# dschrempf/mcmc-date

Measured on AMD Instinct MI355X. Metric: MVN log-likelihood evals/sec (= MCMC steps/sec × chains) at N=256 nodes, higher is better.
Workload: dtype f64; 1 GPU; synthetic 256-dimensional MVN (dense random SPD Sigma, seed 256), 512 chains per GPU, kind=logpdf; n=256, chains_per_gpu=512, kernel=logpdf, launch=hipGraph replay, swap_period=0, parallelism=chains sharded x1, no data-path collective, form=sweep

## Files before the change

mcmc-date_amd/csrc/k_logpdf.hip:

```cpp
#include "mvn_device.hpp"
#include "stripe_device.hpp"

namespace mcd {

template <int R, int BT, int CW, int LW, int FS>
__global__ void __launch_bounds__(64 * (CW + LW)) k_logpdf(const double* __restrict__ F, const double* __restrict__ mu,
                                                           const double* __restrict__ invdiag, const double* __restrict__ X, int64_t ldx,
                                                           int64_t batch, int n, int ncols, double* __restrict__ ll, double c, double logdet)
{
    MCD_KERNEL_HEAD_FS(FS)
    MCD_ACC_DECL
    MCD_T(0);
    if (wave >= CW) {
        const int lw = wave - CW;
        fwd_loader_role<R, LW, FS>(F, ring, lw, lane, ncols MCD_ACC_ARGS);
        MCD_T(3);
        MCD_ACC_FLUSH(5);
        return;
    }
    const MvnView M(mu, invdiag, n, c, logdet);
    double d[R][BT];
    load_rawx<R, BT, FS == 2>(d, M, X, ldx, b0, batch, lane);
    MCD_T(1);
    lds_barrier();
// ... 2 lines not shown
    MCD_T(3);
    finish_ll<R, BT>(d, M, b0, batch, ll, lane);
    MCD_T(4);
    MCD_ACC_FLUSH(5);
}

template <int R, int S, bool SH, int SC>
__global__ void __launch_bounds__(64 * S) k_logpdf_stripe(const double* __restrict__ Fw, const double* __restrict__ mu,
                                                          const double* __restrict__ invdiag, const double* __restrict__ X, int64_t ldx,
                                                          int64_t batch, int n, int ncols, double* __restrict__ ll, double c, double logdet)
{
    __shared__ d2 ring[SH ? Stripe<R, S>::D3 : Stripe<R, S>::D2];
    const int lane = threadIdx.x & 63;
    const int wave = __builtin_amdgcn_readfirstlane(threadIdx.x >> 6);
    MCD_T(0);
    const MvnView M(mu, invdiag, n, c, logdet);
    stripe_dispatch<R, S, 0, SH, SC>(wave, Fw, ring, M, X, ldx, (int64_t)blockIdx.x * 2, batch, ncols, ll, lane);
}

template <int R, int S>
__global__ void __launch_bounds__(64 * S) k_logpdf_stripe_fin(const double* __restrict__ Fw, const double* __restrict__ mu,
                                                              const double* __restrict__ invdiag, const double* __restrict__ X, int64_t ldx,
                                                              int64_t batch, int n, int ncols, double* __restrict__ ll, double c, double logdet)
{
    static_assert(kStripeArgC == 8 * 8, "c follows Fw, mu, invdiag, X, ldx, batch, {n, ncols} and ll");
    __shared__ d2 ring[Stripe<R, S>::D3];
    const int lane = threadIdx.x & 63;
    const int wave = __builtin_amdgcn_readfirstlane(threadIdx.x >> 6);
    MCD_T(0);
    const MvnView M(mu, invdiag, n, 0.0, 0.0);
    stripe_dispatch_fin<R, S, 0>(wave, Fw, ring, M, X, ldx, (int64_t)blockIdx.x * 2, batch, ncols, ll, lane);
}

template <int R, bool SH, int SC>
static void launch_stripe_sh(const MvnDev& M, const double* X, int64_t ldx, int64_t batch, double* ll, hipStream_t st)
{
    hipLaunchKernelGGL((k_logpdf_stripe<R, kStripeWaves, SH, SC>), dim3((unsigned)((batch + 1) / 2)), dim3(64 * kStripeWaves), 0, st, M.Fw, M.mu,
                       M.invdiag, X, ldx, batch, M.n, M.ncols, ll, M.c, M.logdet);
}
template <int R>
static void launch_stripe(const MvnDev& M, const double* X, int64_t ldx, int64_t batch, double* ll, hipStream_t st)
{
    const int pro = opt_or(OPT_STRIPE_PROLOGUE, kStripePrologueDefault), sched = opt_or(OPT_STRIPE_SCHED, kStripeSchedDefault);
    const int sc = stripe_schedule(pro, sched, R, M.ncols);
    if (sc < 0) launch_stripe_sh<R, false, 0>(M, X, ldx, batch, ll, st);
    else if (stripe_finish(pro, sched, opt_or(OPT_STRIPE_FINISH, kStripeFinishDefault), R, M.ncols) != 0)
        hipLaunchKernelGGL((k_logpdf_stripe_fin<R, kStripeWaves>), dim3((unsigned)((batch + 1) / 2)), dim3(64 * kStripeWaves), 0, st, M.Fw, M.mu,
                           M.invdiag, X, ldx, batch, M.n, M.ncols, ll, M.c, M.logdet);
    else if (sc == 2) launch_stripe_sh<R, true, 2>(M, X, ldx, batch, ll, st);
    else if (sc == 1) launch_stripe_sh<R, true, 1>(M, X, ldx, batch, ll, st);
    else launch_stripe_sh<R, true, 0>(M, X, ldx, batch, ll, st);
}

template <int R, int BT, int CW, int LW, int FS>
static void launch_fs(const MvnDev& M, const double* X, int64_t ldx, int64_t batch, double* ll, hipStream_t st)
{
    const int64_t per_wg = (int64_t)CW * BT;
    const unsigned grid = (unsigned)((batch + per_wg - 1) / per_wg);
    hipLaunchKernelGGL((k_logpdf<R, BT, CW, LW, FS>), dim3(grid), dim3(64 * (CW + LW)), 0, st, fwd_stream_ptr(M, FS), M.mu, M.invdiag, X, ldx,
                       batch, M.n, M.ncols, ll, M.c, M.logdet);
}

template <int R, int BT, int CW, int LW>
static void launch_geom(const MvnDev& M, const double* X, int64_t ldx, int64_t batch, double* ll, hipStream_t st)
{
    if constexpr (fwd_stream_compact(R)) {
        constexpr bool INV = CW == 2 && BT == 1;
        const int fs = fwd_stream<R>(CW, INV, INV && logpdf_inverse_window(MvnFacts(M), batch));
        if (fs == 1) return launch_fs<R, BT, CW, LW, 1>(M, X, ldx, batch, ll, st);
        if (fs == 2) return launch_fs<R, BT, CW, LW, 2>(M, X, ldx, batch, ll, st);
        if constexpr (INV)
            if (fs == 3) return launch_stripe<R>(M, X, ldx, batch, ll, st);
    }
    launch_fs<R, BT, CW, LW, 0>(M, X, ldx, batch, ll, st);
}

template <int R>
static hipError_t launch_logpdf_R(const MvnDev& M, const double* X, int64_t ldx, int64_t batch, double* ll, hipStream_t st)
{
// ... 40 lines not shown
```

mcmc-date_amd/csrc/mvn_capi.cpp:

```cpp
#include <hip/hip_runtime.h>

#include <cmath>
#include <cstdarg>
#include <cstdio>
#include <cstring>
#include <memory>
#include <mutex>
#include <string>
#include <vector>

#include "../../include/mcmcdate_mvn.h"
#include "fc_layout.hpp"
#include "host_factor.h"
#include "mvn_kernels.h"

namespace {

thread_local std::string g_last_error;

int fail(int code, const char* fmt, ...)
{
    char buf[512];
    va_list ap;
    va_start(ap, fmt);
// ... 207 lines not shown
        mcd::invert_factor(n, h->L, W);
    }
    h->n = n;
    h->R = mcd::padded_blocks(n);
    h->device = device_id;
    if (h->R < 0) return fail(MCD_ERR_UNSUPPORTED, "mcd_mvn_create: unsupported dimension %d", n);
    if (mat_kind == MCD_MAT_SIGMA_INV) {
        h->logdet = logdet_sigma;
    } else {
        double s = 0.0;
        for (int i = 0; i < n; ++i) s += std::log(h->L[(size_t)i * n + i]);
        h->logdet = 2.0 * s;
    }
    std::vector<double> mu_pad, invdiag, Ft, Ut;
    mcd::pack_factors(n, h->R, h->L, mu_pad, mu, invdiag, Ft, Ut);

    HIP_TRY(hipSetDevice(device_id));
    const size_t NP = (size_t)64 * h->R;
    HIP_TRY(hipMalloc((void**)&h->d_mu, NP * sizeof(double)));
    HIP_TRY(hipMalloc((void**)&h->d_invdiag, NP * sizeof(double)));
    HIP_TRY(hipMalloc((void**)&h->d_Ft, NP * NP * sizeof(double)));
    HIP_TRY(hipMalloc((void**)&h->d_Ut, NP * NP * sizeof(double)));
    HIP_TRY(hipMemcpy(h->d_mu, mu_pad.data(), NP * sizeof(double), hipMemcpyHostToDevice));
    HIP_TRY(hipMemcpy(h->d_invdiag, invdiag.data(), NP * sizeof(double), hipMemcpyHostToDevice));
    HIP_TRY(hipMemcpy(h->d_Ft, Ft.data(), NP * NP * sizeof(double), hipMemcpyHostToDevice));
    HIP_TRY(hipMemcpy(h->d_Ut, Ut.data(), NP * NP * sizeof(double), hipMemcpyHostToDevice));
    if (mcd::fwd_stream_compact(h->R)) {
        std::vector<double> Fc;
        mcd::pack_compact_forward(h->R, Ft, Fc);
        HIP_TRY(hipMalloc((void**)&h->d_Fc, Fc.size() * sizeof(double)));
        HIP_TRY(hipMemcpy(h->d_Fc, Fc.data(), Fc.size() * sizeof(double), hipMemcpyHostToDevice));
        std::vector<double> Fw;
        mcd::pack_inverse_forward(n, h->R, W, Fw);
        HIP_TRY(hipMalloc((void**)&h->d_Fw, Fw.size() * sizeof(double)));
        HIP_TRY(hipMemcpy(h->d_Fw, Fw.data(), Fw.size() * sizeof(double), hipMemcpyHostToDevice));
    }

    const int ch = mcd::sweep_chunk_columns(h->R);
    h->dev.n = n;
    h->dev.R = h->R;
    h->dev.ncols = ((n + ch - 1) / ch) * ch;
    h->dev.c = -(0.9189385332046727417803297364056176 * (double)n);
    h->dev.logdet = h->logdet;
    h->dev.mu = h->d_mu;
    h->dev.invdiag = h->d_invdiag;
    h->dev.Ft = h->d_Ft;
    h->dev.Fc = h->d_Fc;
    h->dev.Fw = h->d_Fw;
    h->dev.Ut = h->d_Ut;
    {
        std::vector<double> Wt, Wtb;
        mcd::pack_w_tiles(n, W, Wt, Wtb);
        HIP_TRY(hipMalloc((void**)&h->d_Wt, Wt.size() * sizeof(double)));
        HIP_TRY(hipMemcpy(h->d_Wt, Wt.data(), Wt.size() * sizeof(double), hipMemcpyHostToDevice));
        HIP_TRY(hipMalloc((void**)&h->d_Wtb, Wtb.size() * sizeof(double)));
        HIP_TRY(hipMemcpy(h->d_Wtb, Wtb.data(), Wtb.size() * sizeof(double), hipMemcpyHostToDevice));
        h->dev.Wt = h->d_Wt;
        h->dev.Wtb = h->d_Wtb;
        if (h->R >= 1) {
            std::vector<double> Wc((size_t)n * NP, 0.0);
            for (int j = 0; j < n; ++j)
                for (int i = j; i < n; ++i) Wc[(size_t)j * NP + i] = W[(size_t)i * n + j];
            HIP_TRY(hipMalloc((void**)&h->d_Wc, Wc.size() * sizeof(double)));
            HIP_TRY(hipMemcpy(h->d_Wc, Wc.data(), Wc.size() * sizeof(double), hipMemcpyHostToDevice));
            h->dev.Wc = h->d_Wc;
        }
        HIP_TRY(mcd::prepare_wide());
        HIP_TRY(mcd::prepare_wide_grad());
// ... 307 lines not shown
```

mcmc-date_amd/csrc/options.cpp:

```cpp
#include "options.h"

#include <atomic>
#include <cstdlib>
#include <cstring>

#include "../../include/mcmcdate_mvn.h"

extern "C" int mcd_set_last_error_(int code, const char* msg);

namespace mcd {
namespace {

const char* const kNames[OPT_COUNT] = {
    "MCD_MH_PER_PHASE", "MCD_MH_SEGMENTS", "MCD_MH_INCREMENTAL", "MCD_MH_PRIOR", "MCD_MH_PRIOR_CACHE", "MCD_MH_STEP_WG", "MCD_MH_CHAIN_LW",
    "MCD_MH_INC_SLOTS", "MCD_MH_SPARSE_SLOTS", "MCD_SPLIT", "MCD_SPLIT_G", "MCD_SPLIT_SCATTER", "MCD_SPLIT_NOROT", "MCD_SPLIT_PROBE", "MCD_GEOM",
    "MCD_WIDE_CT", "MCD_SPARSE_QUAD", "MCD_MH_PRIOR_WAVES", "MCD_LOADERS", "MCD_MH_SEG_TAIL", "MCD_MH_AHEAD_FROM", "MCD_MH_PRIOR_DRAWS",
    "MCD_FSTREAM", "MCD_SPARSE_GRAD_CHAINS", "MCD_STRIPE_PROLOGUE", "MCD_STRIPE_SCHED", "MCD_STRIPE_FINISH"};

struct Table {
    std::atomic<int> v[OPT_COUNT];
    Table()
    {
        for (int i = 0; i < OPT_COUNT; ++i) {
            const char* e = std::getenv(kNames[i]);
            v[i].store((e && *e) ? std::atoi(e) : MCD_OPT_UNSET, std::memory_order_relaxed);
        }
    }
};
Table& table()
{
    static Table t;
    return t;
}
const Table& g_seed_at_load = table();

int find(const char* name)
{
    if (!name) return -1;
    for (int i = 0; i < OPT_COUNT; ++i)
        if (std::strcmp(name, kNames[i]) == 0) return i;
    return -1;
}

}

int opt_get(Option o) { return table().v[o].load(std::memory_order_relaxed); }

namespace {
thread_local unsigned long long t_last_lds = 0;
}
// ... 27 lines not shown
```

mcmc-date_amd/csrc/options.h:

```cpp
#pragma once

namespace mcd {

enum Option {
    OPT_MH_PER_PHASE = 0,
    OPT_MH_SEGMENTS,
    OPT_MH_INCREMENTAL,
    OPT_MH_PRIOR,
    OPT_MH_PRIOR_CACHE,
    OPT_MH_STEP_WG,
    OPT_MH_CHAIN_LW,
    OPT_MH_INC_SLOTS,
    OPT_MH_SPARSE_SLOTS,
    OPT_SPLIT,
    OPT_SPLIT_G,
    OPT_SPLIT_SCATTER,
    OPT_SPLIT_NOROT,
    OPT_SPLIT_PROBE,
    OPT_GEOM,
    OPT_WIDE_CT,
    OPT_SPARSE_QUAD,
    OPT_MH_PRIOR_WAVES,
    OPT_LOADERS,
    OPT_MH_SEG_TAIL,
    OPT_MH_AHEAD_FROM,
    OPT_MH_PRIOR_DRAWS,
    OPT_FSTREAM,
    OPT_SPARSE_GRAD_CHAINS,
    OPT_STRIPE_PROLOGUE,
    OPT_STRIPE_SCHED,
    OPT_STRIPE_FINISH,
    OPT_COUNT
};
constexpr int MCD_OPT_UNSET = -2147483647 - 1;

int opt_get(Option o);
void note_dynamic_lds(unsigned long long bytes);
unsigned long long last_dynamic_lds();
inline bool opt_is(Option o, int v) { return opt_get(o) == v; }
inline int opt_or(Option o, int dflt) { const int v = opt_get(o); return v == MCD_OPT_UNSET ? dflt : v; }

}
```

mcmc-date_amd/csrc/stripe_device.hpp:

```cpp
#pragma once
#include "mvn_device.hpp"
#include "stripe_deal.hpp"
#include "stripe_plan.hpp"

namespace mcd {

#ifndef MCD_STRIPE_WAVES
#define MCD_STRIPE_WAVES 4
#endif
constexpr int kStripeWaves = MCD_STRIPE_WAVES;
#ifndef MCD_STRIPE_AHEAD
#define MCD_STRIPE_AHEAD 12
#endif
constexpr int kStripeAhead = MCD_STRIPE_AHEAD;

template <int R, int S>
struct Stripe {
    static_assert((R == 3 || R == 4) && (S == 4 || S == 8), "stripe kernel: R = 3, 4; S = 4, 8");
    static constexpr int D = 128 / S;
    static constexpr int A = kStripeAhead < D ? kStripeAhead : D;
    static_assert(A >= 1, "MCD_STRIPE_AHEAD");
    static constexpr int ZERO = S * D * 64;
    static constexpr int D2 = ZERO + S * 64;
    static constexpr int EXCH = D2;
// ... 544 lines not shown
        }
    }
    MCD_T(1);
}

template <int R, int S, int W, int I, int NO>
__device__ __forceinline__ void stripe_exchange_put(const double (&xr)[NO + 1][2], const double (&m)[NO + 1], const double (&iv)[NO + 1], unsigned ea,
                                                    int n, int64_t b0, int64_t batch, int lane)
{
    if constexpr (I < NO) {
        constexpr int k = W + I * S;
        const int row = 64 * k + lane;
        double rr[2], tt[2];
#pragma unroll
        for (int c = 0; c < 2; ++c) {
            const double xv = (row < n && b0 + c < batch) ? xr[I][c] : m[I];
            rr[c] = xv - m[I];
            tt[c] = rr[c] * iv[I];
        }
        lds_write16<k * 1024>(ea, d2{rr[0], rr[1]});
        lds_write16<(R + k) * 1024>(ea, d2{tt[0], tt[1]});
        stripe_exchange_put<R, S, W, I + 1, NO>(xr, m, iv, ea, n, b0, batch, lane);
    }
}
template <int R, int Q, int K>
__device__ __forceinline__ void stripe_exchange_get(d2 (&e)[R], unsigned ea)
{
    if constexpr (K < R) {
        lds_read16<(Q * R + K) * 1024>(e[K], ea);
        stripe_exchange_get<R, Q, K + 1>(e, ea);
    }
}

template <int R, int S, int W, bool GETR = true, class Burst>
__device__ __forceinline__ void stripe_prologue_shared(unsigned ea, const MvnView& M, const double* __restrict__ X, int64_t ldx, int64_t b0,
                                                       int64_t batch, double (&r)[R][2], double (&a)[R][2], int lane, Burst burst)
{
    using G = Stripe<R, S>;
    constexpr int PRO = stripe_min(G::A, G::T.n[W]);
    constexpr int NO = W < R ? (R - W + S - 1) / S : 0;
    double xr[NO + 1][2], m[NO + 1], iv[NO + 1];
#pragma unroll
    for (int i = 0; i < NO; ++i) {
        const int row = 64 * (W + i * S) + lane;
        asm_load8(m[i], M.mu + row);
        asm_load8(iv[i], M.invdiag + row);
        const int rc = row < M.n ? row : M.n - 1;
#pragma unroll
        for (int c = 0; c < 2; ++c) {
            const int64_t bc = (b0 + c < batch) ? b0 + c : batch - 1;
            asm_load8(xr[i][c], X + bc * ldx + rc);
        }
    }
    burst();
    asm_wait_vmcnt<PRO>();
#pragma unroll
    for (int i = 0; i < NO; ++i) asm volatile("" : "+v"(m[i]), "+v"(iv[i]), "+v"(xr[i][0]), "+v"(xr[i][1]));
    MCD_T(1);
    stripe_exchange_put<R, S, W, 0, NO>(xr, m, iv, ea, M.n, b0, batch, lane);
    lds_barrier();
    d2 e[R], et[R];
    if constexpr (GETR) stripe_exchange_get<R, 0, 0>(e, ea);
    if constexpr (W == 0) stripe_exchange_get<R, 1, 0>(et, ea);
    if constexpr (GETR) lds_landed<R>(e);
    if constexpr (W == 0) lds_landed<R>(et);
#pragma unroll
    for (int k = 0; k < R; ++k)
#pragma unroll
        for (int c = 0; c < 2; ++c) {
            if constexpr (GETR) r[k][c] = c ? e[k].y : e[k].x;
            if constexpr (W == 0) a[k][c] = c ? et[k].y : et[k].x;
            else a[k][c] = 0.0;
// ... 48 lines not shown
            const double* pw = reinterpret_cast<const double*>(ring + w * D * 64);
#pragma unroll
            for (int k = 0; k < R; ++k)
#pragma unroll
                for (int c = 0; c < 2; ++c) a[k][c] = a[k][c] + pw[(k * 2 + c) * 64 + lane];
        }
        finish_ll<R, 2>(a, M, b0, batch, ll, lane);
        MCD_T(4);
    }
}

#ifndef MCD_STRIPE_FINISH_WAVE
#define MCD_STRIPE_FINISH_WAVE 0
#endif
constexpr int kStripeFinishWave = MCD_STRIPE_FINISH_WAVE;
constexpr int kStripeArgC = 0x40;
typedef unsigned stripe_u4 __attribute__((ext_vector_type(4)));
__device__ __forceinline__ void stripe_args_load(stripe_u4& v)
{
#if defined(__HIP_DEVICE_COMPILE__)
    asm volatile("s_load_dwordx4 %0, %1, %2" : "=&s"(v) : "s"(__builtin_amdgcn_kernarg_segment_ptr()), "n"(kStripeArgC) : "memory");
#endif
}
__device__ __forceinline__ void stripe_args_landed(stripe_u4& v)
{
    asm volatile("s_waitcnt lgkmcnt(0)" : "+s"(v)::"memory");
}
template <int OFF>
__device__ __forceinline__ void lds_read8(double& v, unsigned addr)
{
    static_assert(OFF >= 0 && OFF < 65536, "ds offset");
    asm volatile("ds_read_b64 %0, %1 offset:%2" : "=v"(v) : "v"(addr), "n"(OFF) : "memory");
}
template <int R, int S, int W, int C, int I>
__device__ __forceinline__ void stripe_finish_get(double (&p)[S][R], unsigned pa)
{
    if constexpr (I < S * R) {
        constexpr int w = I / R, k = I % R;
        if constexpr (w != W) lds_read8<(k * 2 + C) * 512>(p[w][k], pa + (unsigned)(w * Stripe<R, S>::D * 1024));
        stripe_finish_get<R, S, W, C, I + 1>(p, pa);
    }
}
template <int R, int S, int W, int C>
__device__ __forceinline__ void stripe_finish_chain(const double (&a)[R][2], unsigned pa, stripe_u4& cl, int64_t b0, int64_t batch,
                                                    double* __restrict__ ll, int lane)
{
    double p[S][R];
    stripe_finish_get<R, S, W, C, 0>(p, pa);
    asm volatile("s_waitcnt lgkmcnt(0)" ::: "memory");
#pragma unroll
    for (int w = 0; w < S; ++w)
#pragma unroll
        for (int k = 0; k < R; ++k)
            if (w != W) asm volatile("" : "+v"(p[w][k]));
    MCD_T(7);
    double s = 0.0;
#pragma unroll
    for (int k = 0; k < R; ++k) {
        double z = W == 0 ? a[k][C] : p[0][k];
#pragma unroll
        for (int w = 1; w < S; ++w) z = z + (w == W ? a[k][C] : p[w][k]);
        s = fma(z, z, s);
    }
    const double q = wave_sum(s);
    stripe_args_landed(cl);
    const double c = __hiloint2double((int)cl.y, (int)cl.x), logdet = __hiloint2double((int)cl.w, (int)cl.z);
    if (lane == 0 && b0 + C < batch) ll[b0 + C] = c + (-0.5) * (logdet + q);
}

template <int R, int S, int W>
__device__ __forceinline__ void stripe_wave_fin(const double* __restrict__ Fw, d2* ring, const MvnView& M, const double* __restrict__ X, int64_t ldx,
                                                int64_t b0, int64_t batch, int ncols, double* __restrict__ ll, int lane)
{
    using G = Stripe<R, S>;
    static_assert(kStripeFinishWave >= 0 && kStripeFinishWave + 2 <= S, "MCD_STRIPE_FINISH_WAVE");
    constexpr int D = G::D, NU = G::T.n[W], PRO = stripe_min(G::A, NU);
    constexpr int C = W - kStripeFinishWave;
    constexpr bool FIN = C == 0 || C == 1;
    stripe_u4 cl;
    if constexpr (FIN) stripe_args_load(cl);
    d2* my = ring + W * D * 64;
// ... 15 lines not shown
    for (int k = 0; k < R; ++k)
#pragma unroll
        for (int c = 0; c < 2; ++c)
            if (c != C) part[(k * 2 + c) * 64 + lane] = a[k][c];
    lds_barrier();
    if constexpr (FIN) {
        MCD_T(6);
        stripe_finish_chain<R, S, W, C>(a, lds_addr(ring) + 8u * (unsigned)lane, cl, b0, batch, ll, lane);
        MCD_T(4);
    }
}
template <int R, int S, int W>
__device__ __forceinline__ void stripe_dispatch_fin(int wave, const double* __restrict__ Fw, d2* ring, const MvnView& M, const double* __restrict__ X,
                                                    int64_t ldx, int64_t b0, int64_t batch, int ncols, double* __restrict__ ll, int lane)
{
    if (wave == W) {
        stripe_wave_fin<R, S, W>(Fw, ring, M, X, ldx, b0, batch, ncols, ll, lane);
    } else {
        if constexpr (W + 1 < S) stripe_dispatch_fin<R, S, W + 1>(wave, Fw, ring, M, X, ldx, b0, batch, ncols, ll, lane);
    }
}

template <int R, int S, int W, bool SH, int SC>
__device__ __forceinline__ void stripe_dispatch(int wave, const double* __restrict__ Fw, d2* ring, const MvnView& M, const double* __restrict__ X,
                                                int64_t ldx, int64_t b0, int64_t batch, int ncols, double* __restrict__ ll, int lane)
{
    if (wave == W) {
        stripe_wave<R, S, W, SH, SC>(Fw, ring, M, X, ldx, b0, batch, ncols, ll, lane);
    } else {
        if constexpr (W + 1 < S) stripe_dispatch<R, S, W + 1, SH, SC>(wave, Fw, ring, M, X, ldx, b0, batch, ncols, ll, lane);
    }
}

}
```

mcmc-date_amd/csrc/stripe_plan.hpp:

```cpp
#pragma once

#include "stripe_deal.hpp"

namespace mcd {

constexpr int kStripeRegSlots = 24;
constexpr int kStripeMaxGroups = 32;
constexpr int kStripeBaseSpan = 8192, kStripeBaseBias = 4096;

struct StripePlan {
    int n, lead, pro, D, A;
    int kind[kStripeMaxUnits];
    int slot[kStripeMaxUnits];
    int base[kStripeMaxUnits];
    int imm[kStripeMaxUnits];
    int group[kStripeMaxUnits];
    int ng;
    int gci[kStripeMaxGroups], gdiag[kStripeMaxGroups];
    int gbeg[kStripeMaxGroups], gend[kStripeMaxGroups];
    int gpre[kStripeMaxGroups];
    int gwait[kStripeMaxGroups];
    int gpost[kStripeMaxGroups];
};

// ... 97 lines not shown
        issued = upto;
    };
    issue(p.pro, -1, -1);
    if (p.lead + issued >= 64) return 3;
    for (int g = 0; g < p.ng && !fail; ++g) {
        issue(p.gpre[g], g - 2, g - 1);
        if (issued - landed >= 64) return 3;
        if (issued < p.gend[g] || p.gwait[g] != issued - p.gend[g] || p.gwait[g] > 63) return 2;
        landed = p.gend[g];
        issue(p.gpost[g], g - 1, g);
        if (issued - landed >= 64) return 3;
    }
    if (fail) return fail;
    return issued == p.n ? 0 : 8;
}

constexpr bool stripe_plans_cover(int R, int S, int A)
{
    int seen[256] = {};
    const StripeDeal d = stripe_deal(R, S);
    for (int w = 0; w < S; ++w) {
        const StripePlan p = stripe_plan(R, S, w, A);
        if (stripe_plan_check(p, R, S, w) != 0) return false;
        for (int u = 0; u < p.n; ++u) {
            const int unit = p.kind[u] ? (p.base[u] + p.imm[u]) / 1024 : d.unit[w][u];
            if (unit < 0 || unit >= fc_total_units(R) || seen[unit]++) return false;
        }
    }
    for (int i = 0; i < fc_total_units(R); ++i)
        if (seen[i] != 1) return false;
    return true;
}

}
```

mcmc-date_amd/csrc/sweep_launch.cpp:

```cpp
#include "sweep_groups.hpp"
#include "stripe_deal.hpp"
#include "stripe_plan.hpp"
#include <stdlib.h>
#include <atomic>

namespace mcd {

int sweep_chunk_columns(int R)
{
    return 2 * ((R == 1) ? 32 : (R == 2) ? 16 : (R <= 4) ? 8 : 4);
}

int wide_chain_tiles(int64_t batch)
{
    const int force = opt_or(OPT_WIDE_CT, 0);
    if (force == 1 || force == 2 || force == 4) return force;
    return batch <= 256 * 16 ? 1 : 2;
}

static std::atomic<int> g_form{getenv("MCD_WIDE") ? (atoi(getenv("MCD_WIDE")) ? 2 : 1) : 0};

int set_logpdf_form(int form) { return g_form.exchange(form); }

int effective_form(const MvnDev& M)
// ... 216 lines not shown
    if ((R != 3 && R != 4) || (S != 4 && S != 8) || w < 0 || w >= S) return -1;
    const mcd::StripeDeal d = mcd::stripe_deal(R, S);
    int np = 0;
    auto put = [&](int ci, int p, int pos, int units) {
        if (np < cap) {
            int* q = piece + 5 * np;
            q[0] = ci, q[1] = p, q[2] = d.unit[w][pos], q[3] = units, q[4] = pos;
        }
        ++np;
    };
    for (int ci = 0; ci < mcd::fc_nchunk(R) && 16 * ci < ncols; ++ci) {
        if (d.diag_pos[w][ci] >= 0) put(ci, -1, d.diag_pos[w][ci], mcd::fc_diag_units(R, ci % mcd::fc_cpb(R)));
        for (int p = 0; p < mcd::fc_cp(R); ++p)
            if (d.pair_pos[w][ci][p] >= 0) put(ci, p, d.pair_pos[w][ci][p], R - 1 - ci / mcd::fc_cpb(R));
    }
    return np <= cap ? np : -2;
}

extern "C" int mcd_stripe_schedule_selftest_(int R, int ncols)
{
    if (R != 3 && R != 4) return -2;
    return mcd::stripe_schedule(mcd::opt_or(mcd::OPT_STRIPE_PROLOGUE, mcd::kStripePrologueDefault),
                                mcd::opt_or(mcd::OPT_STRIPE_SCHED, mcd::kStripeSchedDefault), R, ncols);
}

extern "C" int mcd_stripe_finish_selftest_(int R, int ncols)
{
    if (R != 3 && R != 4) return -2;
    return mcd::stripe_finish(mcd::opt_or(mcd::OPT_STRIPE_PROLOGUE, mcd::kStripePrologueDefault),
                              mcd::opt_or(mcd::OPT_STRIPE_SCHED, mcd::kStripeSchedDefault),
                              mcd::opt_or(mcd::OPT_STRIPE_FINISH, mcd::kStripeFinishDefault), R, ncols);
}

extern "C" int mcd_stripe_plan_selftest_(int R, int S, int w, int A, int* head, int* pos, int cap_pos, int* grp, int cap_grp)
{
    if ((R != 3 && R != 4) || (S != 4 && S != 8) || w < 0 || w >= S || A < 1) return -1;
    const mcd::StripePlan p = mcd::stripe_plan(R, S, w, A);
    const mcd::StripeDeal d = mcd::stripe_deal(R, S);
    if (p.n > cap_pos || p.ng > cap_grp) return -2;
    head[0] = p.n, head[1] = p.ng, head[2] = p.lead, head[3] = p.pro, head[4] = p.D, head[5] = mcd::kStripeRegSlots;
    for (int u = 0; u < p.n; ++u) {
        int* q = pos + 6 * u;
        q[0] = p.kind[u], q[1] = p.slot[u], q[2] = p.base[u], q[3] = p.imm[u], q[4] = d.unit[w][u], q[5] = p.group[u];
    }
    for (int g = 0; g < p.ng; ++g) {
        int* q = grp + 7 * g;
        q[0] = p.gci[g], q[1] = p.gdiag[g], q[2] = p.gbeg[g], q[3] = p.gend[g], q[4] = p.gpre[g], q[5] = p.gwait[g], q[6] = p.gpost[g];
    }
    return mcd::stripe_plan_check(p, R, S, w);
}
```

Measured before the change: 111.3 million evals/s.

## Add register-ring stripe logpdf kernel streaming factor directly into registers

Adds a new stripe kernel variant that loads the inverse-factor tiles from global memory straight into a per-wave register ring, following a compile-time checked issue/wait plan. It uses an LDS ring only for the x broadcast and the final partial-sum handoff. Diagonal parts are loaded per pair, and lanes below a threshold are redirected to a zero pad appended to the Fw buffer. The kernel is selected by default for batch >= 385, which covers the 512-chain workload. It aims to remove the LDS staging round-trip for factor data, at the cost of higher register pressure and a more complex schedule.

Result: faster. 115.8 million evals/s (median of 6 runs) (+4.0%).

```diff
diff --git a/mcmc-date_amd/csrc/k_logpdf.hip b/mcmc-date_amd/csrc/k_logpdf.hip
--- a/mcmc-date_amd/csrc/k_logpdf.hip
+++ b/mcmc-date_amd/csrc/k_logpdf.hip
@@ -58,6 +58,20 @@
     stripe_dispatch_fin<R, S, 0>(wave, Fw, ring, M, X, ldx, (int64_t)blockIdx.x * 2, batch, ncols, ll, lane);
 }
 
+template <int R, int S>
+__global__ void __launch_bounds__(64 * S) k_logpdf_stripe_reg(const double* __restrict__ Fw, const double* __restrict__ mu,
+                                                              const double* __restrict__ invdiag, const double* __restrict__ X, int64_t ldx,
+                                                              int64_t batch, int n, int ncols, double* __restrict__ ll, double c, double logdet)
+{
+    static_assert(kStripeArgC == 8 * 8, "c follows Fw, mu, invdiag, X, ldx, batch, {n, ncols} and ll");
+    __shared__ d2 lds[StripeReg<R, S>::D2];
+    const int lane = threadIdx.x & 63;
+    const int wave = __builtin_amdgcn_readfirstlane(threadIdx.x >> 6);
+    MCD_T(0);
+    const MvnView M(mu, invdiag, n, 0.0, 0.0);
+    stripe_dispatch_reg<R, S, 0>(wave, Fw, lds, M, X, ldx, (int64_t)blockIdx.x * 2, batch, ncols, ll, lane);
+}
+
 template <int R, bool SH, int SC>
 static void launch_stripe_sh(const MvnDev& M, const double* X, int64_t ldx, int64_t batch, double* ll, hipStream_t st)
 {
@@ -68,9 +82,12 @@
 static void launch_stripe(const MvnDev& M, const double* X, int64_t ldx, int64_t batch, double* ll, hipStream_t st)
 {
     const int pro = opt_or(OPT_STRIPE_PROLOGUE, kStripePrologueDefault), sched = opt_or(OPT_STRIPE_SCHED, kStripeSchedDefault);
-    const int sc = stripe_schedule(pro, sched, R, M.ncols);
+    const int sc = stripe_schedule(pro, sched, R, M.ncols), fin = opt_or(OPT_STRIPE_FINISH, kStripeFinishDefault);
     if (sc < 0) launch_stripe_sh<R, false, 0>(M, X, ldx, batch, ll, st);
-    else if (stripe_finish(pro, sched, opt_or(OPT_STRIPE_FINISH, kStripeFinishDefault), R, M.ncols) != 0)
+    else if (stripe_diag(pro, sched, fin, opt_or(OPT_STRIPE_DIAG, stripe_diag_default(batch)), R, M.ncols) != 0)
+        hipLaunchKernelGGL((k_logpdf_stripe_reg<R, kStripeWaves>), dim3((unsigned)((batch + 1) / 2)), dim3(64 * kStripeWaves), 0, st, M.Fw, M.mu,
+                           M.invdiag, X, ldx, batch, M.n, M.ncols, ll, M.c, M.logdet);
+    else if (stripe_finish(pro, sched, fin, R, M.ncols) != 0)
         hipLaunchKernelGGL((k_logpdf_stripe_fin<R, kStripeWaves>), dim3((unsigned)((batch + 1) / 2)), dim3(64 * kStripeWaves), 0, st, M.Fw, M.mu,
                            M.invdiag, X, ldx, batch, M.n, M.ncols, ll, M.c, M.logdet);
     else if (sc == 2) launch_stripe_sh<R, true, 2>(M, X, ldx, batch, ll, st);
diff --git a/mcmc-date_amd/csrc/mvn_capi.cpp b/mcmc-date_amd/csrc/mvn_capi.cpp
--- a/mcmc-date_amd/csrc/mvn_capi.cpp
+++ b/mcmc-date_amd/csrc/mvn_capi.cpp
@@ -263,8 +263,10 @@
         HIP_TRY(hipMemcpy(h->d_Fc, Fc.data(), Fc.size() * sizeof(double), hipMemcpyHostToDevice));
         std::vector<double> Fw;
         mcd::pack_inverse_forward(n, h->R, W, Fw);
-        HIP_TRY(hipMalloc((void**)&h->d_Fw, Fw.size() * sizeof(double)));
-        HIP_TRY(hipMemcpy(h->d_Fw, Fw.data(), Fw.size() * sizeof(double), hipMemcpyHostToDevice));
+        const size_t zero_at = Fw.size();
+        HIP_TRY(hipMalloc((void**)&h->d_Fw, (zero_at + 128) * sizeof(double)));
+        HIP_TRY(hipMemcpy(h->d_Fw, Fw.data(), zero_at * sizeof(double), hipMemcpyHostToDevice));
+        HIP_TRY(hipMemset(h->d_Fw + zero_at, 0, 128 * sizeof(double)));
     }
 
     const int ch = mcd::sweep_chunk_columns(h->R);
diff --git a/mcmc-date_amd/csrc/options.cpp b/mcmc-date_amd/csrc/options.cpp
--- a/mcmc-date_amd/csrc/options.cpp
+++ b/mcmc-date_amd/csrc/options.cpp
@@ -15,7 +15,7 @@
     "MCD_MH_PER_PHASE", "MCD_MH_SEGMENTS", "MCD_MH_INCREMENTAL", "MCD_MH_PRIOR", "MCD_MH_PRIOR_CACHE", "MCD_MH_STEP_WG", "MCD_MH_CHAIN_LW",
     "MCD_MH_INC_SLOTS", "MCD_MH_SPARSE_SLOTS", "MCD_SPLIT", "MCD_SPLIT_G", "MCD_SPLIT_SCATTER", "MCD_SPLIT_NOROT", "MCD_SPLIT_PROBE", "MCD_GEOM",
     "MCD_WIDE_CT", "MCD_SPARSE_QUAD", "MCD_MH_PRIOR_WAVES", "MCD_LOADERS", "MCD_MH_SEG_TAIL", "MCD_MH_AHEAD_FROM", "MCD_MH_PRIOR_DRAWS",
-    "MCD_FSTREAM", "MCD_SPARSE_GRAD_CHAINS", "MCD_STRIPE_PROLOGUE", "MCD_STRIPE_SCHED", "MCD_STRIPE_FINISH"};
+    "MCD_FSTREAM", "MCD_SPARSE_GRAD_CHAINS", "MCD_STRIPE_PROLOGUE", "MCD_STRIPE_SCHED", "MCD_STRIPE_FINISH", "MCD_STRIPE_DIAG"};
 
 struct Table {
     std::atomic<int> v[OPT_COUNT];
diff --git a/mcmc-date_amd/csrc/options.h b/mcmc-date_amd/csrc/options.h
--- a/mcmc-date_amd/csrc/options.h
+++ b/mcmc-date_amd/csrc/options.h
@@ -30,6 +30,7 @@
     OPT_STRIPE_PROLOGUE,
     OPT_STRIPE_SCHED,
     OPT_STRIPE_FINISH,
+    OPT_STRIPE_DIAG,
     OPT_COUNT
 };
 constexpr int MCD_OPT_UNSET = -2147483647 - 1;
diff --git a/mcmc-date_amd/csrc/stripe_device.hpp b/mcmc-date_amd/csrc/stripe_device.hpp
--- a/mcmc-date_amd/csrc/stripe_device.hpp
+++ b/mcmc-date_amd/csrc/stripe_device.hpp
@@ -600,12 +600,12 @@
     }
 }
 
-template <int R, int S, int W, bool GETR = true, class Burst>
+template <int R, int S, int W, bool GETR = true, int BURST = -1, class Burst>
 __device__ __forceinline__ void stripe_prologue_shared(unsigned ea, const MvnView& M, const double* __restrict__ X, int64_t ldx, int64_t b0,
                                                        int64_t batch, double (&r)[R][2], double (&a)[R][2], int lane, Burst burst)
 {
     using G = Stripe<R, S>;
-    constexpr int PRO = stripe_min(G::A, G::T.n[W]);
+    constexpr int PRO = BURST >= 0 ? BURST : stripe_min(G::A, G::T.n[W]);
     constexpr int NO = W < R ? (R - W + S - 1) / S : 0;
     double xr[NO + 1][2], m[NO + 1], iv[NO + 1];
 #pragma unroll
@@ -720,21 +720,21 @@
     static_assert(OFF >= 0 && OFF < 65536, "ds offset");
     asm volatile("ds_read_b64 %0, %1 offset:%2" : "=v"(v) : "v"(addr), "n"(OFF) : "memory");
 }
-template <int R, int S, int W, int C, int I>
+template <int R, int S, int W, int C, int I, int REGION = Stripe<R, S>::D * 1024>
 __device__ __forceinline__ void stripe_finish_get(double (&p)[S][R], unsigned pa)
 {
     if constexpr (I < S * R) {
         constexpr int w = I / R, k = I % R;
-        if constexpr (w != W) lds_read8<(k * 2 + C) * 512>(p[w][k], pa + (unsigned)(w * Stripe<R, S>::D * 1024));
-        stripe_finish_get<R, S, W, C, I + 1>(p, pa);
-    }
-}
-template <int R, int S, int W, int C>
+        if constexpr (w != W) lds_read8<(k * 2 + C) * 512>(p[w][k], pa + (unsigned)(w * REGION));
+        stripe_finish_get<R, S, W, C, I + 1, REGION>(p, pa);
+    }
+}
+template <int R, int S, int W, int C, int REGION = Stripe<R, S>::D * 1024>
 __device__ __forceinline__ void stripe_finish_chain(const double (&a)[R][2], unsigned pa, stripe_u4& cl, int64_t b0, int64_t batch,
                                                     double* __restrict__ ll, int lane)
 {
     double p[S][R];
-    stripe_finish_get<R, S, W, C, 0>(p, pa);
+    stripe_finish_get<R, S, W, C, 0, REGION>(p, pa);
     asm volatile("s_waitcnt lgkmcnt(0)" ::: "memory");
 #pragma unroll
     for (int w = 0; w < S; ++w)
@@ -816,4 +816,176 @@
     }
 }
 
-}
+template <int R, int S>
+struct StripeReg {
+    static constexpr int EXCH = 0;
+    static constexpr int HAND = 2 * R * 64;
+    static constexpr int REGION = R * 1024;
+    static constexpr int D2 = HAND + S * R * 64;
+    static_assert(stripe_reg_plans_cover(R, S, kStripeRegAhead), "stripe register plan: every off-diagonal unit and every (part, pair) once");
+};
+template <int R, int S, int W>
+struct StripeRegPlanOf {
+    static constexpr StripeRegPlan P = stripe_reg_plan(R, S, W, kStripeRegAhead);
+    static_assert(stripe_reg_plan_check(P, R, S, W) == 0, "stripe register plan: waits, outstanding operations, slot reuse, immediates, lane addresses");
+};
+template <int R, int S, int W, int U0, int U1>
+__device__ __forceinline__ void stripe_reg_issue(const double* __restrict__ Fw, int lane, unsigned voff, d2 (&RR)[kStripeRegRing])
+{
+    if constexpr (U0 < U1) {
+        constexpr const StripeRegPlan& P = StripeRegPlanOf<R, S, W>::P;
+        constexpr int slot = P.slot[U0], base = P.base[U0];
+        if constexpr (P.thr[U0] < 0) {
+            stripe_load_reg<P.imm[U0]>(RR[slot], voff, reinterpret_cast<const char*>(Fw) + base);
+        } else {
+            constexpr int thr = P.thr[U0];
+            constexpr unsigned zoff = (unsigned)P.zoff[U0];
+            unsigned v = lane > thr ? voff : zoff;
+            asm volatile("" : "+v"(v));
+            stripe_load_reg<P.imm[U0]>(RR[slot], v, reinterpret_cast<const char*>(Fw) + base);
+        }
+        stripe_reg_issue<R, S, W, U0 + 1, U1>(Fw, lane, voff, RR);
+    }
+}
+template <int R, int S, int W, int U0, int U1>
+__device__ __forceinline__ void stripe_reg_pin(d2 (&RR)[kStripeRegRing])
+{
+    if constexpr (U0 < U1) {
+        constexpr int slot = StripeRegPlanOf<R, S, W>::P.slot[U0];
+        asm volatile("" : "+v"(RR[slot]));
+        stripe_reg_pin<R, S, W, U0 + 1, U1>(RR);
+    }
+}
+template <int R, int S, int W, int GI, int P_, int NREAD, int NZ>
+__device__ __forceinline__ void stripe_reg_pairs_apply(const d2 (&RR)[kStripeRegRing], const d2 (&z)[16], double (&a)[R][2])
+{
+    if constexpr (P_ < 8) {
+        constexpr const StripeRegPlan& P = StripeRegPlanOf<R, S, W>::P;
+        constexpr int CI = P.gci[GI], JB = CI / 4, NKO = R - 1 - JB, pos = Stripe<R, S>::T.pair_pos[W][CI][P_];
+        if constexpr (pos >= 0) {
+            constexpr int u0 = P.gbeg[GI] + NREAD, s0 = P.slot[u0];
+            static_assert(u0 + NKO <= P.gend[GI] && P.unit[u0] == Stripe<R, S>::T.unit[W][pos] && P.thr[u0] < 0, "a pair's requests");
+#pragma unroll
+            for (int h = 0; h < 2; ++h)
+#pragma unroll
+                for (int k = 0; k < NKO; ++k) {
+                    const d2& l = RR[(s0 + k) % kStripeRegRing];
+#pragma unroll
+                    for (int b = 0; b < 2; ++b) a[JB + 1 + k][b] = fma(h ? l.y : l.x, b ? z[NZ + h].y : z[NZ + h].x, a[JB + 1 + k][b]);
+                }
+            stripe_reg_pairs_apply<R, S, W, GI, P_ + 1, NREAD + NKO, NZ + 2>(RR, z, a);
+        } else {
+            stripe_reg_pairs_apply<R, S, W, GI, P_ + 1, NREAD, NZ>(RR, z, a);
+        }
+    }
+}
+template <int R, int S, int W, int GI>
+__device__ __forceinline__ void stripe_reg_apply(const d2 (&RR)[kStripeRegRing], const d2 (&z)[16], double (&a)[R][2])
+{
+    constexpr const StripeRegPlan& P = StripeRegPlanOf<R, S, W>::P;
+    constexpr int JB = P.gci[GI] / 4;
+    if constexpr (P.gdiag[GI] != 0) {
+        static_assert(P.gend[GI] - P.gbeg[GI] == 8 && P.pair[P.gbeg[GI]] == 0, "a part's requests");
+        constexpr int s0 = P.slot[P.gbeg[GI]];
+#pragma unroll
+        for (int p = 0; p < 8; ++p) {
+            const d2& l = RR[(s0 + p) % kStripeRegRing];
+#pragma unroll
+            for (int h = 0; h < 2; ++h)
+#pragma unroll
+                for (int b = 0; b < 2; ++b) a[JB][b] = fma(h ? l.y : l.x, b ? z[2 * p + h].y : z[2 * p + h].x, a[JB][b]);
+        }
+    } else {
+        stripe_reg_pairs_apply<R, S, W, GI, 0, 0, 0>(RR, z, a);
+    }
+}
+template <int R, int S, int W, int GI>
+__device__ __forceinline__ void stripe_reg_ahead(const double* __restrict__ Fw, unsigned xa, unsigned voff, double (&a)[R][2],
+                                                 d2 (&RR)[kStripeRegRing], d2 (&Z)[2][16], int lane)
+{
+    constexpr const StripeRegPlan& P = StripeRegPlanOf<R, S, W>::P;
+    constexpr StripeGroups Q = stripe_groups<R, S, W>();
+    static_assert(Q.n == P.ng && Q.ci[GI] == P.gci[GI] && Q.diag[GI] == P.gdiag[GI], "the plan's groups are the schedule's");
+    if constexpr (GI + 1 < P.ng) {
+        constexpr int N = GI + 1;
+        stripe_group_bcast<R, S, W, N>(Z[N & 1], xa);
+        MCD_SB;
+        stripe_reg_apply<R, S, W, GI>(RR, Z[GI & 1], a);
+        MCD_SB;
+        stripe_reg_issue<R, S, W, P.gpost[GI], P.gpre[N]>(Fw, lane, voff, RR);
+        asm_wait_vmcnt<P.gwait[N]>();
+        stripe_reg_pin<R, S, W, P.gbeg[N], P.gend[N]>(RR);
+        lds_landed<stripe_group_cols<R, S, W, N>()>(Z[N & 1]);
+        stripe_reg_issue<R, S, W, P.gpre[N], P.gpost[N]>(Fw, lane, voff, RR);
+        stripe_reg_ahead<R, S, W, N>(Fw, xa, voff, a, RR, Z, lane);
+    } else {
+        stripe_reg_apply<R, S, W, GI>(RR, Z[GI & 1], a);
+    }
+}
+template <int R, int S, int W>
+__device__ __forceinline__ void stripe_reg_sched(const double* __restrict__ Fw, unsigned xa, unsigned voff, double (&a)[R][2],
+                                                 d2 (&RR)[kStripeRegRing], int lane, int ncols)
+{
+    constexpr const StripeRegPlan& P = StripeRegPlanOf<R, S, W>::P;
+    if (ncols <= 0) {
+        MCD_SB;
+        asm_wait_vmcnt<0>();
+        MCD_SB;
+        return;
+    }
+    d2 Z[2][16];
+    stripe_group_bcast<R, S, W, 0>(Z[0], xa);
+    stripe_reg_issue<R, S, W, P.pro, P.gpre[0]>(Fw, lane, voff, RR);
+    asm_wait_vmcnt<P.gwait[0]>();
+    MCD_T(2);
+    stripe_reg_pin<R, S, W, P.gbeg[0], P.gend[0]>(RR);
+    lds_landed<stripe_group_cols<R, S, W, 0>()>(Z[0]);
+    stripe_reg_issue<R, S, W, P.gpre[0], P.gpost[0]>(Fw, lane, voff, RR);
+    stripe_reg_ahead<R, S, W, 0>(Fw, xa, voff, a, RR, Z, lane);
+}
+template <int R, int S, int W>
+__device__ __forceinline__ void stripe_wave_reg(const double* __restrict__ Fw, d2* lds, const MvnView& M, const double* __restrict__ X, int64_t ldx,
+                                                int64_t b0, int64_t batch, int ncols, double* __restrict__ ll, int lane)
+{
+    using G = StripeReg<R, S>;
+    constexpr const StripeRegPlan& P = StripeRegPlanOf<R, S, W>::P;
+    static_assert(kStripeFinishWave >= 0 && kStripeFinishWave + 2 <= S, "MCD_STRIPE_FINISH_WAVE");
+    constexpr int C = W - kStripeFinishWave;
+    constexpr bool FIN = C == 0 || C == 1;
+    stripe_u4 cl;
+    if constexpr (FIN) stripe_args_load(cl);
+    double r[R][2], a[R][2];
+    const unsigned voff = 16u * (unsigned)lane, xa = lds_addr(lds + G::EXCH);
+    d2 RR[kStripeRegRing];
+    stripe_prologue_shared<R, S, W, false, P.pro>(xa + voff, M, X, ldx, b0, batch, r, a, lane,
+                                                  [&]() __attribute__((always_inline)) { stripe_reg_issue<R, S, W, 0, P.pro>(Fw, lane, voff, RR); });
+    stripe_reg_sched<R, S, W>(Fw, xa, voff, a, RR, lane, ncols);
+    MCD_T(3);
+    MCD_SB;
+    asm_wait_vmcnt<0>();
+    MCD_SB;
+    double* part = reinterpret_cast<double*>(lds + G::HAND + W * R * 64);
+#pragma unroll
+    for (int k = 0; k < R; ++k)
+#pragma unroll
+        for (int c = 0; c < 2; ++c)
+            if (c != C) part[(k * 2 + c) * 64 + lane] = a[k][c];
+    lds_barrier();
+    if constexpr (FIN) {
+        MCD_T(6);
+        stripe_finish_chain<R, S, W, C, G::REGION>(a, lds_addr(lds + G::HAND) + 8u * (unsigned)lane, cl, b0, batch, ll, lane);
+        MCD_T(4);
+    }
+}
+template <int R, int S, int W>
+__device__ __forceinline__ void stripe_dispatch_reg(int wave, const double* __restrict__ Fw, d2* lds, const MvnView& M, const double* __restrict__ X,
+                                                    int64_t ldx, int64_t b0, int64_t batch, int ncols, double* __restrict__ ll, int lane)
+{
+    if (wave == W) {
+        stripe_wave_reg<R, S, W>(Fw, lds, M, X, ldx, b0, batch, ncols, ll, lane);
+    } else {
+        if constexpr (W + 1 < S) stripe_dispatch_reg<R, S, W + 1>(wave, Fw, lds, M, X, ldx, b0, batch, ncols, ll, lane);
+    }
+}
+
+}
diff --git a/mcmc-date_amd/csrc/stripe_plan.hpp b/mcmc-date_amd/csrc/stripe_plan.hpp
--- a/mcmc-date_amd/csrc/stripe_plan.hpp
+++ b/mcmc-date_amd/csrc/stripe_plan.hpp
@@ -153,4 +153,178 @@
     return true;
 }
 
-}
+constexpr int kStripeRegRing = 32;
+constexpr int kStripeRegMaxReq = 96;
+#ifndef MCD_STRIPE_REG_AHEAD
+#define MCD_STRIPE_REG_AHEAD 12
+#endif
+constexpr int kStripeRegAhead = MCD_STRIPE_REG_AHEAD;
+struct StripeRegPlan {
+    int n, lead, pro, A, NS;
+    int slot[kStripeRegMaxReq];
+    int base[kStripeRegMaxReq], imm[kStripeRegMaxReq];
+    int thr[kStripeRegMaxReq];
+    int zoff[kStripeRegMaxReq];
+    int unit[kStripeRegMaxReq], pair[kStripeRegMaxReq];
+    int group[kStripeRegMaxReq];
+    int ng;
+    int gci[kStripeMaxGroups], gdiag[kStripeMaxGroups];
+    int gbeg[kStripeMaxGroups], gend[kStripeMaxGroups];
+    int gpre[kStripeMaxGroups], gwait[kStripeMaxGroups], gpost[kStripeMaxGroups];
+};
+
+constexpr int stripe_reg_zero(int R) { return fc_total_units(R) * 1024; }
+constexpr int stripe_reg_pair_off(int R, int lc, int p) { return 16 * (fc_diag_start(R, lc, p) - (2 * (lc * fc_cp(R) + p) + 1)); }
+
+constexpr unsigned stripe_reg_lane_voff(const StripeRegPlan& p, int u, int l)
+{
+    return l > p.thr[u] ? 16u * (unsigned)l : (unsigned)p.zoff[u];
+}
+
+constexpr StripeRegPlan stripe_reg_plan(int R, int S, int W, int A)
+{
+    StripeRegPlan p{};
+    const StripeDeal d = stripe_deal(R, S);
+    const int CPB = fc_cpb(R), CP = fc_cp(R);
+    p.NS = kStripeRegRing;
+    p.lead = W < R ? 4 * ((R - W + S - 1) / S) : 0;
+    int u = 0;
+    for (int ci = 0; ci < fc_nchunk(R); ++ci) {
+        const int lc = ci % CPB, nko = R - 1 - ci / CPB;
+        if (d.diag_pos[W][ci] >= 0) {
+            const int g = p.ng++, part = d.unit[W][d.diag_pos[W][ci]] * 1024;
+            int lo = stripe_reg_pair_off(R, lc, 0), hi = lo;
+            for (int q = 1; q < CP; ++q) {
+                lo = stripe_plan_min(lo, stripe_reg_pair_off(R, lc, q));
+                hi = stripe_plan_max(hi, stripe_reg_pair_off(R, lc, q));
+            }
+            const int bias = stripe_plan_max(0, (lo + hi) / 2 / 16 * 16);
+            p.gci[g] = ci, p.gdiag[g] = 1, p.gbeg[g] = u;
+            for (int q = 0; q < CP; ++q, ++u) {
+                p.group[u] = g, p.unit[u] = part / 1024, p.pair[u] = q;
+                p.thr[u] = 2 * (lc * CP + q);
+                p.base[u] = part + bias;
+                p.imm[u] = stripe_reg_pair_off(R, lc, q) - bias;
+                p.zoff[u] = stripe_reg_zero(R) - (p.base[u] + p.imm[u]);
+            }
+            p.gend[g] = u;
+        }
+        int g = -1;
+        for (int q = 0; q < CP; ++q)
+            if (d.pair_pos[W][ci][q] >= 0) {
+                if (g < 0) {
+                    g = p.ng++;
+                    p.gci[g] = ci, p.gdiag[g] = 0, p.gbeg[g] = u;
+                }
+                for (int k = 0; k < nko; ++k, ++u) {
+                    const int unit = d.unit[W][d.pair_pos[W][ci][q] + k];
+                    p.group[u] = g, p.unit[u] = unit, p.pair[u] = -1, p.thr[u] = -1, p.zoff[u] = 0;
+                    p.base[u] = unit * 1024 / kStripeBaseSpan * kStripeBaseSpan + kStripeBaseBias;
+                    p.imm[u] = unit * 1024 - p.base[u];
+                }
+                p.gend[g] = u;
+            }
+    }
+    p.n = u;
+    p.A = stripe_plan_min(A, p.NS);
+    p.pro = stripe_plan_min(p.A, p.n);
+    for (int i = 0; i < p.n; ++i) p.slot[i] = i % p.NS;
+    int issued = p.pro;
+    for (int g = 0; g < p.ng; ++g) {
+        p.gpre[g] = stripe_plan_max(issued, p.gend[g]);
+        p.gwait[g] = p.gpre[g] - p.gend[g];
+        p.gpost[g] = stripe_plan_max(p.gpre[g], stripe_plan_min(p.n, p.gend[g] + p.A));
+        issued = p.gpost[g];
+    }
+    return p;
+}
+
+constexpr int stripe_reg_plan_check(const StripeRegPlan& p, int R, int S, int W)
+{
+    const StripeDeal d = stripe_deal(R, S);
+    const int CPB = fc_cpb(R), CP = fc_cp(R), total = fc_total_units(R), zero = total * 1024;
+    if (p.n < 1 || p.n > kStripeRegMaxReq || p.ng < 1 || p.ng > kStripeMaxGroups || p.gbeg[0] != 0 || p.gend[p.ng - 1] != p.n) return 1;
+    if (p.NS < 1 || p.NS > kStripeRegRing) return 8;
+    for (int g = 0; g < p.ng; ++g) {
+        if (p.gend[g] <= p.gbeg[g] || (g > 0 && p.gbeg[g] != p.gend[g - 1])) return 1;
+        if (p.gend[g] - p.gbeg[g] > p.NS) return 8;
+        if (p.gdiag[g] && p.gend[g] - p.gbeg[g] != CP) return 1;
+        for (int u = p.gbeg[g]; u < p.gend[g]; ++u) {
+            if (p.group[u] != g) return 1;
+            if (p.gdiag[g] ? p.pair[u] != u - p.gbeg[g] || p.thr[u] < 0 : p.pair[u] != -1 || p.thr[u] != -1) return 1;
+        }
+    }
+    for (int u = 0; u < p.n; ++u) {
+        if (p.imm[u] < -4096 || p.imm[u] > 4095 || p.base[u] < 0) return 5;
+        if (p.slot[u] < 0 || p.slot[u] >= p.NS) return 6;
+        if (p.unit[u] < 0 || p.unit[u] >= total) return 5;
+        if (p.thr[u] < 0) {
+            if (p.base[u] + p.imm[u] != p.unit[u] * 1024) return 5;
+            continue;
+        }
+        const int ci = p.gci[p.group[u]], lc = ci % CPB, q = p.pair[u], pl = lc * CP + q;
+        if (d.diag_pos[W][ci] < 0 || p.unit[u] != fc_chunk_base(R, ci) || p.thr[u] != 2 * pl) return 9;
+        const int part = p.unit[u] * 1024, bytes = fc_diag_units(R, lc) * 1024, first = fc_diag_start(R, lc, q) - (2 * pl + 1);
+        if (p.zoff[u] < 0) return 9;
+        for (int l = 0; l < 64; ++l) {
+            const long long at = (long long)p.base[u] + p.imm[u] + (long long)stripe_reg_lane_voff(p, u, l);
+            if (l > p.thr[u]) {
+                if (at != part + 16 * (first + l) || at < part || at + 16 > part + bytes) return 9;
+            } else if (at != zero) return 9;
+        }
+    }
+    int owner[kStripeRegRing] = {};
+    for (int i = 0; i < kStripeRegRing; ++i) owner[i] = -1;
+    int issued = 0, landed = 0, fail = 0;
+    auto issue = [&](int upto, int applied) {
+        if (upto < issued || upto > p.n) fail = fail ? fail : 4;
+        for (int u = issued; u < upto && !fail; ++u) {
+            if (owner[p.slot[u]] >= 0 && owner[p.slot[u]] > applied) fail = 6;
+            owner[p.slot[u]] = p.group[u];
+        }
+        issued = upto;
+    };
+    issue(p.pro, -1);
+    if (p.lead + issued >= 64) return 3;
+    for (int g = 0; g < p.ng && !fail; ++g) {
+        issue(p.gpre[g], g - 1);
+        if (issued - landed >= 64) return 3;
+        if (issued < p.gend[g] || p.gwait[g] != issued - p.gend[g] || p.gwait[g] > 63) return 2;
+        landed = p.gend[g];
+        issue(p.gpost[g], g - 1);
+        if (issued - landed >= 64) return 3;
+    }
+    if (fail) return fail;
+    return issued == p.n ? 0 : 8;
+}
+
+constexpr bool stripe_reg_plans_cover(int R, int S, int A)
+{
+    int seen[256] = {}, seen_pair[16][8] = {};
+    for (int w = 0; w < S; ++w) {
+        const StripeRegPlan p = stripe_reg_plan(R, S, w, A);
+        if (stripe_reg_plan_check(p, R, S, w) != 0) return false;
+        for (int u = 0; u < p.n; ++u) {
+            if (p.thr[u] < 0) {
+                if (seen[p.unit[u]]++) return false;
+            } else if (seen_pair[p.gci[p.group[u]]][p.pair[u]]++) return false;
+        }
+    }
+    for (int ci = 0; ci < fc_nchunk(R); ++ci) {
+        const int b = fc_chunk_base(R, ci), du = fc_diag_units(R, ci % fc_cpb(R));
+        for (int q = 0; q < fc_cp(R); ++q)
+            if (seen_pair[ci][q] != 1) return false;
+        for (int i = 0; i < fc_chunk_units(R, ci); ++i)
+            if (seen[b + i] != (i < du ? 0 : 1)) return false;
+    }
+    return true;
+}
+
+constexpr int kStripeDiagFrom = 385;
+constexpr int stripe_diag_default(long long batch) { return batch >= kStripeDiagFrom ? 1 : 0; }
+constexpr int stripe_diag(int prologue, int sched, int finish, int diag, int R, int ncols)
+{
+    return stripe_finish(prologue, sched, finish, R, ncols) == 1 && diag != 0 ? 1 : 0;
+}
+
+}
diff --git a/mcmc-date_amd/csrc/sweep_launch.cpp b/mcmc-date_amd/csrc/sweep_launch.cpp
--- a/mcmc-date_amd/csrc/sweep_launch.cpp
+++ b/mcmc-date_amd/csrc/sweep_launch.cpp
@@ -272,6 +272,34 @@
                               mcd::opt_or(mcd::OPT_STRIPE_FINISH, mcd::kStripeFinishDefault), R, ncols);
 }
 
+extern "C" int mcd_stripe_diag_batch_selftest_(int R, int ncols, long long batch)
+{
+    if (R != 3 && R != 4) return -2;
+    return mcd::stripe_diag(mcd::opt_or(mcd::OPT_STRIPE_PROLOGUE, mcd::kStripePrologueDefault),
+                            mcd::opt_or(mcd::OPT_STRIPE_SCHED, mcd::kStripeSchedDefault),
+                            mcd::opt_or(mcd::OPT_STRIPE_FINISH, mcd::kStripeFinishDefault),
+                            mcd::opt_or(mcd::OPT_STRIPE_DIAG, mcd::stripe_diag_default(batch)), R, ncols);
+}
+extern "C" int mcd_stripe_diag_selftest_(int R, int ncols) { return mcd_stripe_diag_batch_selftest_(R, ncols, 512); }
+
+extern "C" int mcd_stripe_regplan_selftest_(int R, int S, int w, int A, int* head, int* pos, int cap_pos, int* grp, int cap_grp, unsigned* lanes)
+{
+    if ((R != 3 && R != 4) || (S != 4 && S != 8) || w < 0 || w >= S || A < 0) return -1;
+    const mcd::StripeRegPlan p = mcd::stripe_reg_plan(R, S, w, A ? A : mcd::kStripeRegAhead);
+    if (p.n > cap_pos || p.ng > cap_grp) return -2;
+    head[0] = p.n, head[1] = p.ng, head[2] = p.lead, head[3] = p.pro, head[4] = p.NS, head[5] = p.A, head[6] = mcd::stripe_reg_zero(R);
+    for (int u = 0; u < p.n; ++u) {
+        int* q = pos + 8 * u;
+        q[0] = p.slot[u], q[1] = p.base[u], q[2] = p.imm[u], q[3] = p.thr[u], q[4] = p.zoff[u], q[5] = p.unit[u], q[6] = p.pair[u], q[7] = p.group[u];
+        for (int l = 0; lanes && l < 64; ++l) lanes[64 * u + l] = mcd::stripe_reg_lane_voff(p, u, l);
+    }
+    for (int g = 0; g < p.ng; ++g) {
+        int* q = grp + 7 * g;
+        q[0] = p.gci[g], q[1] = p.gdiag[g], q[2] = p.gbeg[g], q[3] = p.gend[g], q[4] = p.gpre[g], q[5] = p.gwait[g], q[6] = p.gpost[g];
+    }
+    return mcd::stripe_reg_plan_check(p, R, S, w);
+}
+
 extern "C" int mcd_stripe_plan_selftest_(int R, int S, int w, int A, int* head, int* pos, int cap_pos, int* grp, int cap_grp)
 {
     if ((R != 3 && R != 4) || (S != 4 && S != 8) || w < 0 || w >= S || A < 1) return -1;
```
